# Iheckzza/FeatureMatching

Hardware: AMD Instinct MI355X
Metric: image-pairs/sec at 640x480 (coarse corr + dual-softmax mutual-NN + fine window refinement) (higher is better)
Workload: dtype i8 screening + f32 exact; 1 GPU; 640x480 pair, C=256 @1/8 (L=S=4800), Cf=64 @1/2, 5x5 fine window, 'peaky' descriptors; launch=hipGraph replay, concurrent_streams=4, fine_maps_layout=nchw

## Files before the change

featurematching_amd/csrc/fine.hip:

```cpp
#include "fm_device.h"
#include "fm_fine_device.h"
#include "fm_maps_device.h"

namespace fm {

__device__ __forceinline__ int xcd_contiguous(int bid, int n) {
  const int q = n >> 3, rem = n & 7, x = bid & 7, y = bid >> 3;
  return (x < rem ? x * (q + 1) : rem * (q + 1) + (x - rem) * q) + y;
}

typedef _Float16 half8 __attribute__((ext_vector_type(8)));
typedef float f32x16 __attribute__((ext_vector_type(16)));

constexpr float kMergeWgtScale = 4096.f;
__device__ __forceinline__ float merge_act_scale(float amax) {
  const unsigned bits = __float_as_uint(amax);
  const int e = (int)((bits >> 23) & 0xffu);
  int k = 140 - e;
  if (e == 255) k = 0;
  k = k > 40 ? 40 : (k < -100 ? -100 : k);
  return __uint_as_float((unsigned)(127 + k) << 23);
}
template <int W>
__device__ __forceinline__ void wave_merge_tile(float* tile, int lane, const half8* __restrict__ wpack,
                                                const float* __restrict__ ctx_row) {
  constexpr int WW = W * W, PITCH = 68, MT = (WW + 31) / 32;
  const int r = lane & 31, h = lane >> 5;
  const float c0 = ctx_row[r], c1 = ctx_row[32 + r];
  half8 bhi[2][4], blo[2][4];
#pragma unroll
  for (int nt = 0; nt < 2; ++nt)
#pragma unroll
    for (int ks = 0; ks < 4; ++ks) {
      bhi[nt][ks] = wpack[((nt * 4 + ks) * 2 + 0) * 64 + lane];
      blo[nt][ks] = wpack[((nt * 4 + ks) * 2 + 1) * 64 + lane];
    }
  float amax = 0.f;
#pragma unroll
  for (int mt = 0; mt < MT; ++mt) {
    const int row = min(32 * mt + r, WW - 1);
#pragma unroll
    for (int ks = 0; ks < 4; ++ks) {
      const float4 p = *reinterpret_cast<const float4*>(tile + row * PITCH + ks * 16 + 8 * h);
      const float4 q = *reinterpret_cast<const float4*>(tile + row * PITCH + ks * 16 + 8 * h + 4);
      amax = fmaxf(amax, fmaxf(fmaxf(fmaxf(fabsf(p.x), fabsf(p.y)), fmaxf(fabsf(p.z), fabsf(p.w))),
                               fmaxf(fmaxf(fabsf(q.x), fabsf(q.y)), fmaxf(fabsf(q.z), fabsf(q.w)))));
    }
  }
#pragma unroll
  for (int m = 32; m >= 1; m >>= 1) amax = fmaxf(amax, __shfl_xor(amax, m));
  const float act_scale = merge_act_scale(amax);
  half8 ahi[MT][4], alo[MT][4];
#pragma unroll
  for (int mt = 0; mt < MT; ++mt) {
    const int row = min(32 * mt + r, WW - 1);
#pragma unroll
    for (int ks = 0; ks < 4; ++ks) {
      const float4 p = *reinterpret_cast<const float4*>(tile + row * PITCH + ks * 16 + 8 * h);
      const float4 q = *reinterpret_cast<const float4*>(tile + row * PITCH + ks * 16 + 8 * h + 4);
      const float x[8] = {p.x, p.y, p.z, p.w, q.x, q.y, q.z, q.w};
#pragma unroll
      for (int e = 0; e < 8; ++e) {
        const float xs = x[e] * act_scale;
        const _Float16 hh = (_Float16)xs;
        ahi[mt][ks][e] = hh;
        alo[mt][ks][e] = (_Float16)(xs - (float)hh);
      }
    }
  }
  __builtin_amdgcn_wave_barrier();
  const float inv_scale = (1.0f / act_scale) * (1.0f / kMergeWgtScale);
#pragma unroll
  for (int mt = 0; mt < MT; ++mt) {
#pragma unroll
    for (int nt = 0; nt < 2; ++nt) {
      f32x16 acc;
#pragma unroll
      for (int g = 0; g < 16; ++g) acc[g] = (nt ? c1 : c0) * (act_scale * kMergeWgtScale);
#pragma unroll
      for (int ks = 0; ks < 4; ++ks) {
        acc = __builtin_amdgcn_mfma_f32_32x32x16_f16(ahi[mt][ks], bhi[nt][ks], acc, 0, 0, 0);
        acc = __builtin_amdgcn_mfma_f32_32x32x16_f16(alo[mt][ks], bhi[nt][ks], acc, 0, 0, 0);
        acc = __builtin_amdgcn_mfma_f32_32x32x16_f16(ahi[mt][ks], blo[nt][ks], acc, 0, 0, 0);
      }
#pragma unroll
      for (int g = 0; g < 16; ++g) {
        const int row = 32 * mt + (g & 3) + 8 * (g >> 2) + 4 * h;
        if (row < WW) tile[row * PITCH + 32 * nt + r] = acc[g] * inv_scale;
      }
    }
  }
  __builtin_amdgcn_wave_barrier();
}

template <int W>
__device__ __forceinline__ void wave_load_window64(const float* src, int Hf, int Wf, int oy, int ox, float* tile, int lane) {
  constexpr int CF = 64, WW = W * W, PITCH = CF + 4;
  constexpr int SLOTS = W == 5 ? 32 : 64, CPI = 64 / SLOTS, NLOAD = CF / CPI;
  static_assert(W == 5 || W == 7, "position decode below is for W in {5,7}");
  const int rem = lane & (SLOTS - 1), hi = lane / SLOTS;
  const int wy = W == 5 ? (rem * 13) >> 6 : (rem * 37) >> 8;
  const int wx = rem - wy * W;
  const int y = oy + wy, x = ox + wx;
  const bool ok = rem < WW && y >= 0 && y < Hf && x >= 0 && x < Wf;
  const __amdgpu_buffer_rsrc_t rsrc =
      __builtin_amdgcn_make_buffer_rsrc(const_cast<float*>(src), 0, CF * Hf * Wf * 4, 0x00020000);
  const unsigned voff = ok ? (unsigned)((hi * Hf + y) * Wf + x) * 4u : 0x80000000u;
  const int step = Hf * Wf * 4 * CPI;
  float v[NLOAD];
#pragma unroll
  for (int it = 0; it < NLOAD; ++it) {
#ifndef FM_ABL_G_NOLOAD
    v[it] = __builtin_bit_cast(float, __builtin_amdgcn_raw_buffer_load_b32(rsrc, voff, it * step, 0));
#else
    v[it] = 0.f;
#endif
  }
  float* slot = tile + rem * PITCH + hi;
#pragma unroll
  for (int it = 0; it < NLOAD; ++it)
    if (rem < WW) slot[it * CPI] = v[it];
  __builtin_amdgcn_wave_barrier();
}

template <int W>
__device__ __forceinline__ void wave_store_tile64(const float* tile, float* __restrict__ dst, int lane) {
  constexpr int CF = 64, WW = W * W, TOTAL = CF * WW, PITCH = CF + 4;
  float4* dst4 = reinterpret_cast<float4*>(dst);
#pragma unroll
  for (int it = 0; it < (TOTAL / 4 + 63) / 64; ++it) {
    const int idx = it * 64 + lane;
    if (idx < TOTAL / 4) {
      const float4 q = *reinterpret_cast<const float4*>(tile + (idx >> 4) * PITCH + (idx & 15) * 4);
#ifdef FM_ABL_G_NOSTORE
      if (q.x == 1.2345e-30f) dst4[idx] = q;
#else
      dst4[idx] = q;
#endif
    }
  }
  __builtin_amdgcn_wave_barrier();
}

template <int W, bool MERGE = false>
__device__ __forceinline__ void wave_copy_window64(const float* src, int Hf, int Wf, int oy, int ox,
                                                   float* __restrict__ dst, float* tile, int lane,
                                                   const half8* __restrict__ wpack = nullptr,
                                                   const float* __restrict__ ctx_row = nullptr) {
  wave_load_window64<W>(src, Hf, Wf, oy, ox, tile, lane);
  if (MERGE) wave_merge_tile<W>(tile, lane, wpack, ctx_row);
  wave_store_tile64<W>(tile, dst, lane);
}

constexpr int kGatherTileFloats(int W) { return W * W * 68; }

template <int W, bool MERGE>
__global__ __launch_bounds__(256) void k_gather_nchw64(const float* __restrict__ feat, int Hf, int Wf, int stride,
                                                       int pad, int w_c, const int64_t* __restrict__ b_ids,
                                                       const int64_t* __restrict__ ids,
                                                       const int32_t* __restrict__ d_count, int m_max,
                                                       float* __restrict__ out, const half8* __restrict__ wpack,
                                                       const float* __restrict__ ctx, int ctx_cells) {
  constexpr int CF = 64, TOTAL = CF * W * W;
  __shared__ __attribute__((aligned(16))) float tile[4 * kGatherTileFloats(W)];
  const int lane = threadIdx.x & 63, wv = __builtin_amdgcn_readfirstlane(threadIdx.x >> 6);
  const int M = d_count ? min(d_count[0], m_max) : m_max;
  const int per = (M + 7) >> 3;
  const int slot = (int)(blockIdx.x >> 3) * 4 + wv;
  const int m = (blockIdx.x & 7) * per + slot;
  if (slot >= per || m >= M) return;
  const int b = __builtin_amdgcn_readfirstlane((int)b_ids[m]);
  const int id = __builtin_amdgcn_readfirstlane((int)ids[m]);
  const int cy = id / w_c;
  wave_copy_window64<W, MERGE>(feat + (long)b * CF * Hf * Wf, Hf, Wf, cy * stride - pad, (id - cy * w_c) * stride - pad,
                               out + (long)m * TOTAL, tile + wv * kGatherTileFloats(W), lane, wpack,
                               MERGE ? ctx + ((long)b * ctx_cells + id) * CF : nullptr);
}

struct CellImage {
  const float* feat; int Hf, Wf, w_c, cells, total_cells;
  const int32_t* cell_to_match; int cell_pitch; const int32_t* ties;
  const int64_t* ids; float* out; const float* ctx;
};
struct CellArgs {
  CellImage im[2];
  int stride, pad, m_max;
  const int64_t* b_ids; const int32_t* d_count; const half8* wpack;
};

template <int W, bool MERGE>
__global__ __launch_bounds__(256) void k_gather_cellorder64(CellArgs a) {
  constexpr int CF = 64, TOTAL = CF * W * W;
  __shared__ __attribute__((aligned(16))) float tile_all[4 * kGatherTileFloats(W)];
  const CellImage& I = a.im[blockIdx.y];
  const int lane = threadIdx.x & 63, wv = __builtin_amdgcn_readfirstlane(threadIdx.x >> 6);
  float* tile = tile_all + wv * kGatherTileFloats(W);
  const int M = a.d_count ? min(a.d_count[0], a.m_max) : a.m_max;
  const int nties = I.ties[0];
  const int lid = xcd_contiguous(blockIdx.x, gridDim.x) * 4 + wv;
  int jm = -1, jb = 0, jcell = 0;
  if (lid < I.total_cells) {
    const int b = lid / I.cells, cell = lid - b * I.cells;
    const int m = I.cell_to_match[(long)b * I.cell_pitch + cell] - 1;
    if (m >= 0 && m < M) { jm = m; jb = b; jcell = cell; }
  }
  const int gwave = blockIdx.x * 4 + wv, nwaves = gridDim.x * 4;
  const int mode = nties == 0 ? 0 : (nties <= kTieCap ? 1 : 2);
  int q = gwave;
  const int chunk = (M + nwaves - 1) / nwaves;
  int scan = gwave * chunk;
  const int scan_end = min(M, scan + chunk);
  for (;;) {
    if (jm >= 0) {
      jm = __builtin_amdgcn_readfirstlane(jm); jb = __builtin_amdgcn_readfirstlane(jb);
      jcell = __builtin_amdgcn_readfirstlane(jcell);
      const int cy = jcell / I.w_c;
      wave_copy_window64<W, MERGE>(I.feat + (long)jb * CF * I.Hf * I.Wf, I.Hf, I.Wf, cy * a.stride - a.pad,
                                   (jcell - cy * I.w_c) * a.stride - a.pad, I.out + (long)jm * TOTAL, tile, lane,
                                   a.wpack, MERGE ? I.ctx + ((long)jb * I.cells + jcell) * CF : nullptr);
    }
    jm = -1;
    if (mode == 0) break;
    if (mode == 1) {
      if (q >= nties) break;
      const int m = I.ties[1 + q];
      q += nwaves;
      if (m >= 0 && m < M) { jm = m; jb = (int)a.b_ids[m]; jcell = (int)I.ids[m]; }
    } else {
      if (scan >= scan_end) break;
      const int m = scan++;
      const int mb = (int)a.b_ids[m], id = (int)I.ids[m];
      if (I.cell_to_match[(long)mb * I.cell_pitch + id] != m + 1) { jm = m; jb = mb; jcell = id; }
    }
  }
}

template <int DT> struct MapElem { using type = float; };
template <> struct MapElem<FM_F16> { using type = unsigned short; };
template <> struct MapElem<FM_BF16> { using type = unsigned short; };
template <int DT>
__device__ __forceinline__ float map_value(const typename MapElem<DT>::type* p, long i) {
  if constexpr (DT == FM_F32) return p[i];
  else return half_bits_to_float(p[i], DT);
}

template <int DT>
__global__ __launch_bounds__(256) void k_gather_nchw(const typename MapElem<DT>::type* __restrict__ feat, int Cf, int Hf, int Wf, int W,
                                                     int stride, int pad, int w_c, const int64_t* __restrict__ b_ids,
                                                     const int64_t* __restrict__ ids, const int32_t* __restrict__ d_count,
                                                     int m_max, float* __restrict__ out) {
  extern __shared__ __attribute__((aligned(16))) float tile[];
  const int m = blockIdx.x;
  const int M = d_count ? min(d_count[0], m_max) : m_max;
  if (m >= M) return;
  const int WW = W * W;
  const int b = (int)b_ids[m];
  const int id = (int)ids[m];
  const int oy = (id / w_c) * stride - pad;
  const int ox = (id % w_c) * stride - pad;
  const typename MapElem<DT>::type* src = feat + (long)b * Cf * Hf * Wf;
  const int total = Cf * WW;
  for (int idx = threadIdx.x; idx < total; idx += 256) {
    const int c = idx / WW;
    const int rem = idx - c * WW;
    const int wy = rem / W, wx = rem - wy * W;
    const int y = oy + wy, x = ox + wx;
    float v = 0.f;
    if (y >= 0 && y < Hf && x >= 0 && x < Wf) v = map_value<DT>(src, ((long)c * Hf + y) * Wf + x);
    tile[rem * (Cf + 1) + c] = v;
  }
  __syncthreads();
  float* dst = out + (long)m * total;
  for (int idx = threadIdx.x; idx < total; idx += 256) {
    const int rpos = idx / Cf;
    const int c = idx - rpos * Cf;
    dst[idx] = tile[rpos * (Cf + 1) + c];
  }
}

template <int DT>
__global__ __launch_bounds__(256) void k_gather_nhwc(const typename MapElem<DT>::type* __restrict__ feat, int Cf, int Hf, int Wf, int W,
                                                     int stride, int pad, int w_c, const int64_t* __restrict__ b_ids,
                                                     const int64_t* __restrict__ ids, const int32_t* __restrict__ d_count,
                                                     int m_max, float* __restrict__ out) {
  const int m = blockIdx.x;
  const int M = d_count ? min(d_count[0], m_max) : m_max;
  if (m >= M) return;
  const int WW = W * W;
  const int b = (int)b_ids[m];
  const int id = (int)ids[m];
  const int oy = (id / w_c) * stride - pad;
  const int ox = (id % w_c) * stride - pad;
  const int c4 = Cf / 4;
  const typename MapElem<DT>::type* src = feat + (long)b * Hf * Wf * Cf;
  float4* dst = reinterpret_cast<float4*>(out + (long)m * WW * Cf);
  for (int idx = threadIdx.x; idx < WW * c4; idx += 256) {
    const int rpos = idx / c4;
    const int c = idx - rpos * c4;
    const int wy = rpos / W, wx = rpos - wy * W;
    const int y = oy + wy, x = ox + wx;
    float4 v = make_float4(0.f, 0.f, 0.f, 0.f);
    if (y >= 0 && y < Hf && x >= 0 && x < Wf) {
      const long e = ((long)y * Wf + x) * c4 + c;
      if constexpr (DT == FM_F32) v = reinterpret_cast<const float4*>(src)[e];
      else v = half4_to_float4(reinterpret_cast<const uint2*>(src)[e], DT);
    }
    dst[idx] = v;
  }
}


template <int W>
__device__ __forceinline__ void soft_argmax2(float sim0, float sim1, int pos, bool on, int lane, float inv_sqrt_c,
                                             float scale_f, float k0x, float k0y, float k1x, float k1y, float* out0,
                                             float* out1) {
  const Heat2 e = heat_exp2(sim0, sim1, on, inv_sqrt_c);
  const float t = heat_sums2<W>(e.e0, e.e1, pos);
  auto sum_k = [&](int k) { return heat_sum(t, k); };
  if (lane == 0) {
    float* const outs[2] = {out0, out1};
    const float kx[2] = {k0x, k1x}, ky[2] = {k0y, k1y};
#pragma unroll
    for (int d = 0; d < 2; ++d) {
      const float inv = 1.0f / sum_k(5 * d);
      const float cx = sum_k(5 * d + 1) * inv, cy = sum_k(5 * d + 2) * inv;
      const float vx = sum_k(5 * d + 3) * inv - cx * cx, vy = sum_k(5 * d + 4) * inv - cy * cy;
      outs[d][0] = kx[d] + (cx * (float)(W / 2) * scale_f + (float)(W / 2));
      outs[d][1] = ky[d] + (cy * (float)(W / 2) * scale_f + (float)(W / 2));
      outs[d][2] = sqrtf(fmaxf(vx, 1e-10f)) + sqrtf(fmaxf(vy, 1e-10f));
    }
  }
}

template <int W>
__device__ __forceinline__ void fine_core(const float (&f0)[W * W], const float (&f1)[W * W], int lane,
                                          const float* __restrict__ mix0, const float* __restrict__ mix1, float k0x,
                                          float k0y, float k1x, float k1y, float scale_f, float* __restrict__ out0,
                                          float* __restrict__ out1) {
  constexpr int WW = W * W;
  constexpr int CF = 64;
  const Mix2 q = fine_mix<W>(f0, f1, mix0, mix1);
  const float q0 = q.q0, q1 = q.q1;

#ifdef FM_ABL_F_NOCOMPUTE
  if (q0 + q1 == 1.2345e-30f) out0[0] = q0;
  return;
#endif
  const float inv_sqrt_c = 1.0f / sqrtf((float)CF);
  constexpr int NP = WW > 32 ? 64 : 32;
  float p[NP];
#pragma unroll
  for (int r = 0; r < NP; ++r) p[r] = r < WW ? q0 * f1[r] : 0.f;
  const float sim0 = transpose_reduce<NP>(p, lane);
#pragma unroll
  for (int r = 0; r < NP; ++r) p[r] = r < WW ? q1 * f0[r] : 0.f;
  const float sim1 = transpose_reduce<NP>(p, lane);

  const int pos = tr_index<NP>(lane);
  const bool on = pos < WW && (NP == 64 || !(lane & 1));
  soft_argmax2<W>(sim0, sim1, pos, on, lane, inv_sqrt_c, scale_f, k0x, k0y, k1x, k1y, out0, out1);
}

template <int W>
__global__ __launch_bounds__(256) void k_fine(const float* __restrict__ win0, const float* __restrict__ win1, int m_max,
                                              const int32_t* __restrict__ d_count, const float* __restrict__ mix0,
                                              const float* __restrict__ mix1, const float* __restrict__ kc0,
                                              const float* __restrict__ kc1, float scale_f, float* __restrict__ out0,
                                              float* __restrict__ out1) {
  constexpr int WW = W * W;
  constexpr int CF = 64;
  const int lane = threadIdx.x & 63;
  const int m = blockIdx.x * 4 + (threadIdx.x >> 6);
  const int M = d_count ? min(d_count[0], m_max) : m_max;
  if (m >= M) return;
  const float* p0 = win0 + (long)m * WW * CF + lane;
  const float* p1 = win1 + (long)m * WW * CF + lane;
  float f0[WW], f1[WW];
#pragma unroll
  for (int r = 0; r < WW; ++r) { f0[r] = __builtin_nontemporal_load(p0 + r * CF); f1[r] = __builtin_nontemporal_load(p1 + r * CF); }
  fine_core<W>(f0, f1, lane, mix0, mix1, kc0[m * 2], kc0[m * 2 + 1], kc1[m * 2], kc1[m * 2 + 1], scale_f,
               out0 + (long)m * 3, out1 + (long)m * 3);
}

template <int W>
__global__ __launch_bounds__(256) void k_gather_nhwc64(const float* __restrict__ feat, int Hf, int Wf, int stride, int pad,
                                                       int w_c, const int64_t* __restrict__ b_ids,
                                                       const int64_t* __restrict__ ids, const int32_t* __restrict__ d_count,
                                                       int m_max, float* __restrict__ out) {
  constexpr int ROW16 = W * 16;
  constexpr int TOTAL16 = W * ROW16;
  constexpr int NIT = (TOTAL16 + 63) / 64;
  const int lane = threadIdx.x & 63, wv = __builtin_amdgcn_readfirstlane(threadIdx.x >> 6);
  const int M = d_count ? min(d_count[0], m_max) : m_max;
  const int per = (M + 7) >> 3;
  const int slot = (int)(blockIdx.x >> 3) * 4 + wv;
  const int m = (blockIdx.x & 7) * per + slot;
  if (slot >= per || m >= M) return;
  const int b = __builtin_amdgcn_readfirstlane((int)b_ids[m]);
  const int id = __builtin_amdgcn_readfirstlane((int)ids[m]);
  const int cy = id / w_c;
  const int oy = cy * stride - pad, ox = (id - cy * w_c) * stride - pad;
  const float4* src = reinterpret_cast<const float4*>(feat + (long)b * Hf * Wf * 64);
  float4* dst = reinterpret_cast<float4*>(out + (long)m * W * W * 64);
  float4 v[NIT];
#pragma unroll
  for (int it = 0; it < NIT; ++it) {
    const int k = it * 64 + lane;
    const int wy = k / ROW16, within = k - wy * ROW16;
    const int y = oy + wy, x = ox + (within >> 4);
    const bool ok = k < TOTAL16 && y >= 0 && y < Hf && x >= 0 && x < Wf;
    const float4 t = src[ok ? ((long)y * Wf + x) * 16 + (within & 15) : 0];
    v[it] = ok ? t : make_float4(0.f, 0.f, 0.f, 0.f);
  }
#pragma unroll
  for (int it = 0; it < NIT; ++it) {
    const int k = it * 64 + lane;
    if (k < TOTAL16) dst[k] = v[it];
  }
}

struct MergeNhwcImage {
  const void* feat; int Hf, Wf, w_c, cells;
  const int64_t* ids; float* out; const float* ctx;
};
struct MergeNhwcArgs {
  MergeNhwcImage im[2];
  int stride, pad, m_max;
  const int64_t* b_ids; const int32_t* d_count; const half8* wpack;
};

template <int W, int DT>
__global__ __launch_bounds__(256) void k_gather_merge_nhwc64(MergeNhwcArgs a) {
  constexpr int WW = W * W, PITCH = 68;
  constexpr int TOTAL16 = WW * 16;
  constexpr int NIT = (TOTAL16 + 63) / 64;
  using Chunk = typename std::conditional<DT == FM_F32, float4, uint2>::type;
  __shared__ __attribute__((aligned(16))) float tile_all[4 * kGatherTileFloats(W)];
  const MergeNhwcImage& I = a.im[blockIdx.y];
  const int lane = threadIdx.x & 63, wv = __builtin_amdgcn_readfirstlane(threadIdx.x >> 6);
  float* tile = tile_all + wv * kGatherTileFloats(W);
  const int M = a.d_count ? min(a.d_count[0], a.m_max) : a.m_max;
  const int per = (M + 7) >> 3;
  const int slot = (int)(blockIdx.x >> 3) * 4 + wv;
  const int m = (blockIdx.x & 7) * per + slot;
  if (slot >= per || m >= M) return;
  const int b = __builtin_amdgcn_readfirstlane((int)a.b_ids[m]);
  const int id = __builtin_amdgcn_readfirstlane((int)I.ids[m]);
  const int cy = id / I.w_c;
  const int oy = cy * a.stride - a.pad, ox = (id - cy * I.w_c) * a.stride - a.pad;
  const Chunk* src = reinterpret_cast<const Chunk*>(I.feat) + (long)b * I.Hf * I.Wf * 16;
  Chunk v[NIT];
#pragma unroll
  for (int it = 0; it < NIT; ++it) {
    const int k = it * 64 + lane;
    const int pos = k >> 4, wy = pos / W;
    const int y = oy + wy, x = ox + (pos - wy * W);
    const bool ok = k < TOTAL16 && y >= 0 && y < I.Hf && x >= 0 && x < I.Wf;
    const Chunk t = src[ok ? ((long)y * I.Wf + x) * 16 + (k & 15) : 0];
    if constexpr (DT == FM_F32) v[it] = ok ? t : make_float4(0.f, 0.f, 0.f, 0.f);
    else v[it] = ok ? t : make_uint2(0u, 0u);
  }
#pragma unroll
  for (int it = 0; it < NIT; ++it) {
    const int k = it * 64 + lane;
    if (k < TOTAL16) {
      float4* slot4 = reinterpret_cast<float4*>(tile + (k >> 4) * PITCH + (k & 15) * 4);
      if constexpr (DT == FM_F32) *slot4 = v[it];
      else *slot4 = half4_to_float4(v[it], DT);
    }
  }
  __builtin_amdgcn_wave_barrier();
  wave_merge_tile<W>(tile, lane, a.wpack, I.ctx + ((long)b * I.cells + id) * 64);
  wave_store_tile64<W>(tile, I.out + (long)m * WW * 64, lane);
}

template <int W, bool NCHW0, int DT = FM_F32>
__global__ __launch_bounds__(256) void k_fine_maps(const float* __restrict__ map0, const float* __restrict__ map1, int Hf0,
                                                   int Wf0, int Hf1, int Wf1, int stride, int pad, int w0c, int w1c,
                                                   const int64_t* __restrict__ b_ids, const int64_t* __restrict__ i_ids,
                                                   const int64_t* __restrict__ j_ids, const int32_t* __restrict__ d_count,
                                                   int m_max, const float* __restrict__ mix0, const float* __restrict__ mix1,
                                                   const float* __restrict__ kc0, const float* __restrict__ kc1, float scale_f,
                                                   float* __restrict__ out0, float* __restrict__ out1) {
  constexpr int WW = W * W;
  const int lane = threadIdx.x & 63, wv = __builtin_amdgcn_readfirstlane(threadIdx.x >> 6);
  const int M = d_count ? min(d_count[0], m_max) : m_max;
  const int per = (M + 7) >> 3;
  __shared__ __attribute__((aligned(16))) float tile_all[NCHW0 ? 4 * kGatherTileFloats(W) : 4];
  for (int slot = (int)(blockIdx.x >> 3) * 4 + wv; slot < per; slot += (int)(gridDim.x >> 3) * 4) {
  const int m = (blockIdx.x & 7) * per + slot;
  if (m >= M) break;
  const int b = __builtin_amdgcn_readfirstlane((int)b_ids[m]);
  const int i = __builtin_amdgcn_readfirstlane((int)i_ids[m]);
  const int j = __builtin_amdgcn_readfirstlane((int)j_ids[m]);
  const int cy0 = i / w0c, cy1 = j / w1c;
  const int oy0 = cy0 * stride - pad, ox0 = (i - cy0 * w0c) * stride - pad;
  const int oy1 = cy1 * stride - pad, ox1 = (j - cy1 * w1c) * stride - pad;
  constexpr int EB = DT == FM_F32 ? 4 : 2;
  constexpr int PXB = 64 * EB;
  static_assert(!(NCHW0 && DT != FM_F32), "half-precision maps are read channels-last");
  const char* base0 = reinterpret_cast<const char*>(map0) + (long)b * Hf0 * Wf0 * PXB;
  const char* base1 = reinterpret_cast<const char*>(map1) + (long)b * Hf1 * Wf1 * PXB;
  unsigned vo0[W], vo1[W];
#pragma unroll
  for (int wx = 0; wx < W; ++wx) {
    const int x0 = ox0 + wx, x1 = ox1 + wx;
    vo0[wx] = x0 >= 0 ? (unsigned)(x0 * PXB + lane * EB) : 0x80000000u;
    vo1[wx] = x1 >= 0 ? (unsigned)(x1 * PXB + lane * EB) : 0x80000000u;
  }
  auto load_elem = [](const __amdgpu_buffer_rsrc_t r, unsigned vo) -> float {
    if constexpr (DT == FM_F32) return __builtin_bit_cast(float, __builtin_amdgcn_raw_buffer_load_b32(r, vo, 0, 0));
    else return half_bits_to_float((unsigned)(unsigned short)__builtin_amdgcn_raw_buffer_load_b16(r, vo, 0, 0), DT);
  };
  float f0[WW], f1[WW];
#pragma unroll
  for (int wy = 0; wy < W; ++wy) {
    const int y0 = oy0 + wy, y1 = oy1 + wy;
    const bool ok0 = y0 >= 0 && y0 < Hf0, ok1 = y1 >= 0 && y1 < Hf1;
    const __amdgpu_buffer_rsrc_t r1 = __builtin_amdgcn_make_buffer_rsrc(
        const_cast<char*>(base1 + (long)(ok1 ? y1 : 0) * Wf1 * PXB), 0, ok1 ? Wf1 * PXB : 0, 0x00020000);
    if (!NCHW0) {
      const __amdgpu_buffer_rsrc_t r0 = __builtin_amdgcn_make_buffer_rsrc(
          const_cast<char*>(base0 + (long)(ok0 ? y0 : 0) * Wf0 * PXB), 0, ok0 ? Wf0 * PXB : 0, 0x00020000);
#pragma unroll
      for (int wx = 0; wx < W; ++wx) f0[wy * W + wx] = load_elem(r0, vo0[wx]);
    }
#pragma unroll
    for (int wx = 0; wx < W; ++wx) f1[wy * W + wx] = load_elem(r1, vo1[wx]);
  }
  if (NCHW0) {
    float* tile = tile_all + wv * kGatherTileFloats(W);
    wave_load_window64<W>(reinterpret_cast<const float*>(base0), Hf0, Wf0, oy0, ox0, tile, lane);
#pragma unroll
    for (int r = 0; r < WW; ++r) f0[r] = tile[r * 68 + lane];
  }
  fine_core<W>(f0, f1, lane, mix0, mix1, kc0[m * 2], kc0[m * 2 + 1], kc1[m * 2], kc1[m * 2 + 1], scale_f,
               out0 + (long)m * 3, out1 + (long)m * 3);
  }
}


template <typename T>
__global__ __launch_bounds__(256) void k_nchw_to_nhwc64(const T* __restrict__ src, T* __restrict__ dst, int Hf, int Wf,
                                                        int N) {
  __shared__ T tile[64 * 65];
  nchw_to_nhwc64_units<T>(src, dst, Hf, Wf, N, tile, blockIdx.x, gridDim.x);
}

}

using namespace fm;

template <bool MERGE>
static void launch_list64(int W, int blocks, hipStream_t st, const float* feat_f, int Hf, int Wf, int stride, int pad,
                          int w_c, const int64_t* b_ids, const int64_t* ids, const int32_t* d_count, int m_max,
                          float* out, const half8* wpack, const float* ctx, int ctx_cells) {
  with_window(W, [&](auto w) {
    hipLaunchKernelGGL((k_gather_nchw64<decltype(w)::value, MERGE>), dim3(blocks), dim3(256), 0, st, feat_f, Hf, Wf, stride,
                       pad, w_c, b_ids, ids, d_count, m_max, out, wpack, ctx, ctx_cells);
  });
}
static CellImage cell_image(const float* feat, int N, int Hf, int Wf, int h_c, int w_c, const int32_t* map, int pitch,
                            const int32_t* ties, const int64_t* ids, float* out, const float* ctx) {
  CellImage im;
  im.feat = feat; im.Hf = Hf; im.Wf = Wf; im.w_c = w_c; im.cells = h_c * w_c; im.total_cells = N * h_c * w_c;
  im.cell_to_match = map; im.cell_pitch = pitch; im.ties = ties; im.ids = ids; im.out = out; im.ctx = ctx;
  return im;
}
static CellArgs cell_args(const CellImage& im0, const CellImage& im1, int stride, int pad, int m_max, const int64_t* b_ids,
                          const int32_t* d_count, const void* packed_w) {
  CellArgs a;
  a.im[0] = im0; a.im[1] = im1;
  a.stride = stride; a.pad = pad; a.m_max = m_max; a.b_ids = b_ids; a.d_count = d_count; a.wpack = (const half8*)packed_w;
  return a;
}
static bool fast_nchw64(int Cf, int Hf, int Wf, int W) {
  return Cf == 64 && (W == 5 || W == 7) && (long)Hf * Wf * 64 * 4 < (1L << 31);
}
static int list_blocks(int m_max) { return 8 * (((m_max + 7) / 8 + 3) / 4); }
constexpr int kFineGridCap = 1 << 20;
static int cell_blocks(long total) { return (int)(((total + 3) / 4 + 7) / 8 * 8); }
static int launch_cells64(int W, int nimg, long total, const CellArgs& a, hipStream_t st) {
  with_window(W, [&](auto w) {
    auto launch = [&](auto merge) {
      hipLaunchKernelGGL((k_gather_cellorder64<decltype(w)::value, decltype(merge)::value>), dim3(cell_blocks(total), nimg),
                         dim3(256), 0, st, a);
    };
    if (a.wpack) launch(std::true_type{});
    else launch(std::false_type{});
  });
  return (int)hipGetLastError();
}

template <int DT>
static void launch_generic_gather(const void* feat_f, int Cf, int Hf, int Wf, int layout, int W, int stride, int pad, int w_c,
                                  const int64_t* b_ids, const int64_t* ids, const int32_t* d_count, int m_max, float* out,
                                  hipStream_t st) {
  using E = typename MapElem<DT>::type;
  if (layout == 0) {
    const size_t smem = (size_t)W * W * (Cf + 1) * sizeof(float);
    hipLaunchKernelGGL(k_gather_nchw<DT>, dim3(m_max), dim3(256), smem, st, (const E*)feat_f, Cf, Hf, Wf, W, stride, pad, w_c,
                       b_ids, ids, d_count, m_max, out);
  } else {
    hipLaunchKernelGGL(k_gather_nhwc<DT>, dim3(m_max), dim3(256), 0, st, (const E*)feat_f, Cf, Hf, Wf, W, stride, pad, w_c,
                       b_ids, ids, d_count, m_max, out);
  }
}

extern "C" int fm_gather_windows_dtype(const void* feat_f, int map_dtype, int N, int Cf, int Hf, int Wf, int layout, int W,
                                       int stride, int pad, int w_c, const int64_t* b_ids, const int64_t* ids,
                                       const int32_t* d_count, int m_max, float* out, void* stream) {
  if (m_max == 0) return FM_OK;
  if (!feat_f || !b_ids || !ids || !out) return FM_E_NULL;
  if (map_dtype != FM_F32 && map_dtype != FM_F16 && map_dtype != FM_BF16) return FM_E_UNSUPPORTED;
  if (!crop_shape_ok(N, Hf, Wf, stride, m_max) || Cf <= 0 || W <= 0 || w_c <= 0) return FM_E_SHAPE;
  if (W > 15 || Cf > 512 || (layout == 1 && Cf % 4) || (layout != 0 && layout != 1)) return FM_E_UNSUPPORTED;
  hipStream_t st = (hipStream_t)stream;
  if (layout == 0 && (size_t)W * W * (Cf + 1) * sizeof(float) > 64 * 1024 &&
      !(map_dtype == FM_F32 && fast_nchw64(Cf, Hf, Wf, W))) return FM_E_UNSUPPORTED;
  if (map_dtype == FM_F32 && layout == 0 && fast_nchw64(Cf, Hf, Wf, W)) {
    launch_list64<false>(W, list_blocks(m_max), st, (const float*)feat_f, Hf, Wf, stride, pad, w_c, b_ids, ids, d_count, m_max,
                         out, nullptr, nullptr, 0);
  } else if (map_dtype == FM_F32 && layout == 1 && Cf == 64 && (W == 5 || W == 7)) {
    with_window(W, [&](auto w) {
      hipLaunchKernelGGL(k_gather_nhwc64<decltype(w)::value>, dim3(list_blocks(m_max)), dim3(256), 0, st,
                         (const float*)feat_f, Hf, Wf, stride, pad, w_c, b_ids, ids, d_count, m_max, out);
    });
  } else if (map_dtype == FM_F32) {
    launch_generic_gather<FM_F32>(feat_f, Cf, Hf, Wf, layout, W, stride, pad, w_c, b_ids, ids, d_count, m_max, out, st);
  } else if (map_dtype == FM_F16) {
    launch_generic_gather<FM_F16>(feat_f, Cf, Hf, Wf, layout, W, stride, pad, w_c, b_ids, ids, d_count, m_max, out, st);
  } else {
    launch_generic_gather<FM_BF16>(feat_f, Cf, Hf, Wf, layout, W, stride, pad, w_c, b_ids, ids, d_count, m_max, out, st);
  }
  return (int)hipGetLastError();
}

extern "C" int fm_gather_windows(const float* feat_f, int N, int Cf, int Hf, int Wf, int layout, int W, int stride,
                                 int pad, int w_c, const int64_t* b_ids, const int64_t* ids, const int32_t* d_count,
                                 int m_max, float* out, void* stream) {
  return fm_gather_windows_dtype(feat_f, FM_F32, N, Cf, Hf, Wf, layout, W, stride, pad, w_c, b_ids, ids, d_count, m_max, out,
                                 stream);
}

extern "C" int fm_gather_windows_cells(const float* feat_f, int N, int Cf, int Hf, int Wf, int W, int stride, int pad,
                                       int h_c, int w_c, const int32_t* cell_to_match, int cell_pitch,
                                       const int32_t* ties, const int64_t* b_ids, const int64_t* ids,
                                       const int32_t* d_count, int m_max, float* out, void* stream) {
  if (m_max == 0) return FM_OK;
  if (!feat_f || !cell_to_match || !ties || !b_ids || !ids || !out) return FM_E_NULL;
  if (!crop_shape_ok(N, Hf, Wf, stride, m_max) || h_c <= 0 || w_c <= 0 || cell_pitch < h_c * w_c) return FM_E_SHAPE;
  if (!fast_nchw64(Cf, Hf, Wf, W)) return FM_E_UNSUPPORTED;
  const CellImage im = cell_image(feat_f, N, Hf, Wf, h_c, w_c, cell_to_match, cell_pitch, ties, ids, out, nullptr);
  return launch_cells64(W, 1, (long)N * h_c * w_c, cell_args(im, im, stride, pad, m_max, b_ids, d_count, nullptr),
                        (hipStream_t)stream);
}

__global__ __launch_bounds__(256) void k_merge_pack(const float* __restrict__ merge_w, half8* __restrict__ packed) {
  const int idx = blockIdx.x * 256 + threadIdx.x;
  if (idx >= 512) return;
  const int lane = idx & 63, ks = (idx >> 6) & 3, nt = idx >> 8;
  const float* src = merge_w + (32 * nt + (lane & 31)) * 128 + 16 * ks + 8 * (lane >> 5);
  half8 hh, ll;
#pragma unroll
  for (int j = 0; j < 8; ++j) {
    float x = src[j] * kMergeWgtScale;
    if (!(fabsf(x) <= 65504.f)) x = __builtin_nanf("");
    hh[j] = (_Float16)x;
    ll[j] = (_Float16)(x - (float)hh[j]);
  }
  packed[((nt * 4 + ks) * 2 + 0) * 64 + lane] = hh;
  packed[((nt * 4 + ks) * 2 + 1) * 64 + lane] = ll;
}

extern "C" int fm_merge_pack_weights(const float* merge_w, int Cf, void* packed, void* stream) {
  if (!merge_w || !packed) return FM_E_NULL;
  if (Cf != 64) return FM_E_UNSUPPORTED;
  hipLaunchKernelGGL(k_merge_pack, dim3(2), dim3(256), 0, (hipStream_t)stream, merge_w, (half8*)packed);
  return (int)hipGetLastError();
}

extern "C" int fm_gather_merge_windows(const float* feat_f, int N, int Cf, int Hf, int Wf, int W, int stride, int pad,
                                       int h_c, int w_c, const int32_t* cell_to_match, int cell_pitch,
                                       const int32_t* ties, const void* packed_w, const float* ctx_bias,
                                       const int64_t* b_ids, const int64_t* ids, const int32_t* d_count, int m_max,
                                       float* out, void* stream) {
  if (m_max == 0) return FM_OK;
  if (!feat_f || !packed_w || !ctx_bias || !b_ids || !ids || !out) return FM_E_NULL;
  if (cell_to_match && !ties) return FM_E_NULL;
  if (!crop_shape_ok(N, Hf, Wf, stride, m_max) || h_c <= 0 || w_c <= 0 || (cell_to_match && cell_pitch < h_c * w_c))
    return FM_E_SHAPE;
  if (!fast_nchw64(Cf, Hf, Wf, W)) return FM_E_UNSUPPORTED;
  hipStream_t st = (hipStream_t)stream;
  if (cell_to_match) {
    const CellImage im = cell_image(feat_f, N, Hf, Wf, h_c, w_c, cell_to_match, cell_pitch, ties, ids, out, ctx_bias);
    return launch_cells64(W, 1, (long)N * h_c * w_c, cell_args(im, im, stride, pad, m_max, b_ids, d_count, packed_w), st);
  }
  launch_list64<true>(W, list_blocks(m_max), st, feat_f, Hf, Wf, stride, pad, w_c, b_ids, ids, d_count, m_max, out,
                      (const half8*)packed_w, ctx_bias, h_c * w_c);
  return (int)hipGetLastError();
}

extern "C" int fm_gather_windows_pair(const float* feat_f0, const float* feat_f1, int N, int Cf, int Hf0, int Wf0,
                                      int Hf1, int Wf1, int W, int stride, int pad, int h0c, int w0c, int h1c, int w1c,
                                      const int32_t* cell0, int pitch0, const int32_t* ties0, const int32_t* cell1,
                                      int pitch1, const int32_t* ties1, const void* packed_w, const float* ctx0,
                                      const float* ctx1, const int64_t* b_ids, const int64_t* i_ids,
                                      const int64_t* j_ids, const int32_t* d_count, int m_max, float* out0,
                                      float* out1, void* stream) {
  if (m_max == 0) return FM_OK;
  if (!feat_f0 || !feat_f1 || !cell0 || !cell1 || !ties0 || !ties1 || !b_ids || !i_ids || !j_ids || !out0 || !out1)
    return FM_E_NULL;
  if (packed_w && (!ctx0 || !ctx1)) return FM_E_NULL;
  if (!crop_shape_ok(N, Hf0, Wf0, stride, m_max) || !crop_shape_ok(N, Hf1, Wf1, stride, m_max) || h0c <= 0 || w0c <= 0 ||
      h1c <= 0 || w1c <= 0 || pitch0 < h0c * w0c || pitch1 < h1c * w1c)
    return FM_E_SHAPE;
  if (!fast_nchw64(Cf, Hf0, Wf0, W) || !fast_nchw64(Cf, Hf1, Wf1, W)) return FM_E_UNSUPPORTED;
  const CellArgs a = cell_args(cell_image(feat_f0, N, Hf0, Wf0, h0c, w0c, cell0, pitch0, ties0, i_ids, out0, ctx0),
                               cell_image(feat_f1, N, Hf1, Wf1, h1c, w1c, cell1, pitch1, ties1, j_ids, out1, ctx1), stride,
                               pad, m_max, b_ids, d_count, packed_w);
  const long t0 = (long)N * h0c * w0c, t1 = (long)N * h1c * w1c;
  return launch_cells64(W, 2, t0 > t1 ? t0 : t1, a, (hipStream_t)stream);
}

static MergeNhwcImage merge_nhwc_image(const void* feat, int Hf, int Wf, int h_c, int w_c, const int64_t* ids, float* out,
                                       const float* ctx) {
  MergeNhwcImage im;
  im.feat = feat; im.Hf = Hf; im.Wf = Wf; im.w_c = w_c; im.cells = h_c * w_c; im.ids = ids; im.out = out; im.ctx = ctx;
  return im;
}

extern "C" int fm_gather_merge_windows_nhwc(const void* feat_f0, const void* feat_f1, int map_dtype, int N, int Cf, int Hf0,
                                            int Wf0, int Hf1, int Wf1, int W, int stride, int pad, int h0c, int w0c,
                                            int h1c, int w1c, const void* packed_w, const float* ctx0, const float* ctx1,
                                            const int64_t* b_ids, const int64_t* i_ids, const int64_t* j_ids,
                                            const int32_t* d_count, int m_max, float* out0, float* out1, void* stream) {
  if (m_max == 0) return FM_OK;
  const bool pair = feat_f1 != nullptr;
  if (!feat_f0 || !packed_w || !ctx0 || !b_ids || !i_ids || !out0) return FM_E_NULL;
  if (pair && (!ctx1 || !j_ids || !out1)) return FM_E_NULL;
  if (!crop_shape_ok(N, Hf0, Wf0, stride, m_max) || h0c <= 0 || w0c <= 0) return FM_E_SHAPE;
  if (pair && (!crop_shape_ok(N, Hf1, Wf1, stride, m_max) || h1c <= 0 || w1c <= 0)) return FM_E_SHAPE;
  if (map_dtype != FM_F32 && map_dtype != FM_F16 && map_dtype != FM_BF16) return FM_E_UNSUPPORTED;
  if (Cf != 64 || (W != 5 && W != 7)) return FM_E_UNSUPPORTED;
  MergeNhwcArgs a;
  a.im[0] = merge_nhwc_image(feat_f0, Hf0, Wf0, h0c, w0c, i_ids, out0, ctx0);
  a.im[1] = pair ? merge_nhwc_image(feat_f1, Hf1, Wf1, h1c, w1c, j_ids, out1, ctx1) : a.im[0];
  a.stride = stride; a.pad = pad; a.m_max = m_max; a.b_ids = b_ids; a.d_count = d_count; a.wpack = (const half8*)packed_w;
  with_window(W, [&](auto w) {
    auto launch = [&](auto dt) {
      hipLaunchKernelGGL((k_gather_merge_nhwc64<decltype(w)::value, decltype(dt)::value>),
                         dim3(list_blocks(m_max), pair ? 2 : 1), dim3(256), 0, (hipStream_t)stream, a);
    };
    if (map_dtype == FM_F16) launch(int_c<FM_F16>{});
    else if (map_dtype == FM_BF16) launch(int_c<FM_BF16>{});
    else launch(int_c<FM_F32>{});
  });
  return (int)hipGetLastError();
}

extern "C" int fm_fine_match(const float* win0, const float* win1, int m_max, const int32_t* d_count, int WW, int Cf,
                             const float* mix0, const float* mix1, const float* mkpts0_c, const float* mkpts1_c,
                             float scale_f, float* out0, float* out1, void* stream) {
  if (m_max == 0) return FM_OK;
  if (!win0 || !win1 || !mix0 || !mix1 || !mkpts0_c || !mkpts1_c || !out0 || !out1) return FM_E_NULL;
  if (m_max < 0) return FM_E_SHAPE;
  if (Cf != 64 || (WW != 25 && WW != 49)) return FM_E_UNSUPPORTED;
  hipStream_t st = (hipStream_t)stream;
  const int blocks = (m_max + 3) / 4;
  with_window(WW == 25 ? 5 : 7, [&](auto w) {
    hipLaunchKernelGGL(k_fine<decltype(w)::value>, dim3(blocks), dim3(256), 0, st, win0, win1, m_max, d_count, mix0, mix1,
                       mkpts0_c, mkpts1_c, scale_f, out0, out1);
  });
  return (int)hipGetLastError();
}

struct FineMapsScratch { Span map[2]; size_t total; };
static FineMapsScratch fine_maps_layout(int N, int Cf, int Hf0, int Wf0, int Hf1, int Wf1, int map_dtype) {
  const size_t elem = map_dtype == FM_F32 ? 4 : 2;
  FineMapsScratch s;
  s.map[0] = {0, map_dtype == FM_F32 ? 0 : (size_t)N * Cf * elem * (size_t)Hf0 * Wf0};
  s.map[1] = {align256(s.map[0].bytes), (size_t)N * Cf * elem * (size_t)Hf1 * Wf1};
  s.total = s.map[1].at + s.map[1].bytes;
  return s;
}

extern "C" size_t fm_fine_maps_scratch_bytes_dtype(int N, int Cf, int Hf0, int Wf0, int Hf1, int Wf1, int layout, int map_dtype) {
  if (layout != 0 || N <= 0 || Cf <= 0 || Hf0 <= 0 || Wf0 <= 0 || Hf1 <= 0 || Wf1 <= 0) return 0;
  return fine_maps_layout(N, Cf, Hf0, Wf0, Hf1, Wf1, map_dtype).total;
}

template <typename T>
static void launch_channels_last_copy(const void* src, void* dst, int N, int Hf, int Wf, int grid_cap, hipStream_t st) {
  const long pieces = (long)((Wf + 63) / 64) * Hf * N;
  hipLaunchKernelGGL(k_nchw_to_nhwc64<T>, dim3((unsigned)(pieces < grid_cap ? pieces : grid_cap)), dim3(256), 0, st,
                     (const T*)src, (T*)dst, Hf, Wf, N);
}
extern "C" size_t fm_fine_maps_scratch_bytes(int N, int Cf, int Hf0, int Wf0, int Hf1, int Wf1, int layout) {
  return fm_fine_maps_scratch_bytes_dtype(N, Cf, Hf0, Wf0, Hf1, Wf1, layout, FM_F32);
}

extern "C" int fm_fine_match_maps_dtype(const void* feat_f0, const void* feat_f1, int map_dtype, int layout, int N, int Cf,
                                        int Hf0, int Wf0, int Hf1, int Wf1, int W, int stride, int pad, int w0c, int w1c,
                                        const int64_t* b_ids, const int64_t* i_ids, const int64_t* j_ids,
                                        const int32_t* d_count, int m_max, const float* mix0, const float* mix1,
                                        const float* mkpts0_c, const float* mkpts1_c, float scale_f, void* scratch,
                                        float* out0, float* out1, void* stream) {
  if (m_max == 0) return FM_OK;
  if (!feat_f0 || !feat_f1 || !b_ids || !i_ids || !j_ids || !mix0 || !mix1 || !mkpts0_c || !mkpts1_c || !out0 || !out1)
    return FM_E_NULL;
  if (!crop_shape_ok(N, Hf0, Wf0, stride, m_max) || !crop_shape_ok(N, Hf1, Wf1, stride, m_max) || w0c <= 0 || w1c <= 0)
    return FM_E_SHAPE;
  if (map_dtype != FM_F32 && map_dtype != FM_F16 && map_dtype != FM_BF16) return FM_E_UNSUPPORTED;
  if ((layout != 0 && layout != 1 && layout != FM_LAYOUT_NCHW_PREPARED) || !fast_nchw64(Cf, Hf0, Wf0, W) ||
      !fast_nchw64(Cf, Hf1, Wf1, W))
    return FM_E_UNSUPPORTED;
  const bool prepared = layout == FM_LAYOUT_NCHW_PREPARED;
  if (prepared && map_dtype != FM_F32) return FM_E_UNSUPPORTED;
  if (prepared) layout = 0;
  if (layout == 0 && !scratch) return FM_E_NULL;
  hipStream_t st = (hipStream_t)stream;
  const float* m0 = (const float*)feat_f0;
  const float* m1 = (const float*)feat_f1;
  int grid_cap = kFineGridCap;
#ifdef FM_TUNE_ENV
  if (const char* e = getenv("FM_FINE_GRID")) grid_cap = atoi(e) > 0 ? atoi(e) / 8 * 8 : kFineGridCap;
#endif
  if (layout == 0) {
    const FineMapsScratch sc = fine_maps_layout(N, Cf, Hf0, Wf0, Hf1, Wf1, map_dtype);
    float* s0 = span_ptr<float>(scratch, sc.map[0]);
    float* s1 = span_ptr<float>(scratch, sc.map[1]);
    if (map_dtype == FM_F32) {
      if (!prepared) launch_channels_last_copy<float>(feat_f1, s1, N, Hf1, Wf1, grid_cap, st);
    } else {
      launch_channels_last_copy<unsigned short>(feat_f0, s0, N, Hf0, Wf0, grid_cap, st);
      launch_channels_last_copy<unsigned short>(feat_f1, s1, N, Hf1, Wf1, grid_cap, st);
      m0 = s0;
    }
    m1 = s1;
  }
  const int blocks = list_blocks(m_max) < grid_cap ? list_blocks(m_max) : grid_cap;
  with_window(W, [&](auto w) {
    auto launch = [&](auto nchw0, auto dt) {
      hipLaunchKernelGGL((k_fine_maps<decltype(w)::value, decltype(nchw0)::value, decltype(dt)::value>), dim3(blocks),
                         dim3(256), 0, st, m0, m1, Hf0, Wf0, Hf1, Wf1, stride, pad, w0c, w1c, b_ids, i_ids, j_ids, d_count,
                         m_max, mix0, mix1, mkpts0_c, mkpts1_c, scale_f, out0, out1);
    };
    if (map_dtype == FM_F16) launch(std::false_type{}, int_c<FM_F16>{});
    else if (map_dtype == FM_BF16) launch(std::false_type{}, int_c<FM_BF16>{});
    else if (layout == 0) launch(std::true_type{}, int_c<FM_F32>{});
    else launch(std::false_type{}, int_c<FM_F32>{});
  });
  return (int)hipGetLastError();
}

extern "C" int fm_fine_match_maps(const float* feat_f0, const float* feat_f1, int layout, int N, int Cf, int Hf0, int Wf0,
                                  int Hf1, int Wf1, int W, int stride, int pad, int w0c, int w1c, const int64_t* b_ids,
                                  const int64_t* i_ids, const int64_t* j_ids, const int32_t* d_count, int m_max,
                                  const float* mix0, const float* mix1, const float* mkpts0_c, const float* mkpts1_c,
                                  float scale_f, void* scratch, float* out0, float* out1, void* stream) {
  return fm_fine_match_maps_dtype(feat_f0, feat_f1, FM_F32, layout, N, Cf, Hf0, Wf0, Hf1, Wf1, W, stride, pad, w0c, w1c,
                                  b_ids, i_ids, j_ids, d_count, m_max, mix0, mix1, mkpts0_c, mkpts1_c, scale_f, scratch,
                                  out0, out1, stream);
}
```

Before: 20370 image-pairs/s.

## Batch adjacent fine matches into shared strip loads for NCHW 5x5 windows

For the NCHW f32 path with a 5x5 window, consecutive matches whose coarse indices are horizontally adjacent in image 0 are processed together as a run. One overlapping strip of the image-0 map is loaded into LDS with 64-bit buffer loads and reused across the run's windows. Runs that fail the adjacency, stride, parity or alignment checks fall back to per-match processing, and the launch grid is sized by the number of runs. The change adds per-wave control flow, a larger LDS tile and more registers for the extra image-1 windows. Any gain depends on how often adjacent matches actually occur.

```diff
diff --git a/featurematching_amd/csrc/fine.hip b/featurematching_amd/csrc/fine.hip
--- a/featurematching_amd/csrc/fine.hip
+++ b/featurematching_amd/csrc/fine.hip
@@ -120,6 +120,44 @@
 #pragma unroll
   for (int it = 0; it < NLOAD; ++it)
     if (rem < WW) slot[it * CPI] = v[it];
+  __builtin_amdgcn_wave_barrier();
+}
+
+constexpr int kRunStride = 4;
+constexpr int kStripPitch = 65;
+constexpr int kStripPixels(int W, int R) { return kRunStride * (R - 1) + W; }
+constexpr int kStripTileFloats(int W, int R) { return W * kStripPixels(W, R) * kStripPitch; }
+
+template <int W, int R>
+__device__ __forceinline__ void wave_load_strip64(const float* src, int Hf, int Wf, int oy, int ox, float* tile, int lane) {
+  constexpr int CF = 64, SP = kStripPixels(W, R), NX2 = (SP + 1) / 2, USED = W * NX2;
+  constexpr int SLOTS = USED <= 32 ? 32 : 64, CPI = 64 / SLOTS, NLOAD = CF / CPI;
+  static_assert(USED <= 64, "one strip of one channel per wave-load at most");
+  const int rem = lane & (SLOTS - 1), hi = lane / SLOTS;
+  const int wy = rem / NX2, k = rem - wy * NX2;
+  const int y = oy + wy, x = ox + 2 * k;
+  const bool ok = rem < USED && y >= 0 && y < Hf && x >= 0 && x + 1 < Wf;
+  const __amdgpu_buffer_rsrc_t rsrc =
+      __builtin_amdgcn_make_buffer_rsrc(const_cast<float*>(src), 0, CF * Hf * Wf * 4, 0x00020000);
+  const unsigned voff = ok ? (unsigned)((hi * Hf + y) * Wf + x) * 4u : 0x80000000u;
+  const int step = Hf * Wf * 4 * CPI;
+  unsigned long long v[NLOAD];
+#pragma unroll
+  for (int it = 0; it < NLOAD; ++it) {
+#ifndef FM_ABL_G_NOLOAD
+    v[it] = __builtin_bit_cast(unsigned long long, __builtin_amdgcn_raw_buffer_load_b64(rsrc, voff, it * step, 0));
+#else
+    v[it] = 0ull;
+#endif
+  }
+  float* slot = tile + (wy * SP + 2 * k) * kStripPitch + hi;
+  const bool second = 2 * k + 1 < SP;
+#pragma unroll
+  for (int it = 0; it < NLOAD; ++it)
+    if (rem < USED) {
+      slot[it * CPI] = __uint_as_float((unsigned)v[it]);
+      if (second) slot[kStripPitch + it * CPI] = __uint_as_float((unsigned)(v[it] >> 32));
+    }
   __builtin_amdgcn_wave_barrier();
 }
 
@@ -474,6 +512,107 @@
   wave_store_tile64<W>(tile, I.out + (long)m * WW * 64, lane);
 }
 
+
+#ifndef FM_FINE_RUN
+#define FM_FINE_RUN 2
+#endif
+constexpr int kFineRun(int W, bool nchw0) { return nchw0 && W == 5 ? FM_FINE_RUN : 1; }
+constexpr int kFineMapsTileFloats(int W, bool nchw0) {
+  return !nchw0 ? 1
+                : (kFineRun(W, nchw0) > 1 && kStripTileFloats(W, kFineRun(W, nchw0)) > kGatherTileFloats(W)
+                       ? kStripTileFloats(W, kFineRun(W, nchw0))
+                       : kGatherTileFloats(W));
+}
+
+struct FineMapsArgs {
+  const float *__restrict__ map0, *__restrict__ map1;
+  int Hf0, Wf0, Hf1, Wf1, stride, pad, w0c, w1c;
+  const int64_t *__restrict__ b_ids, *__restrict__ i_ids, *__restrict__ j_ids;
+  const float *__restrict__ mix0, *__restrict__ mix1, *__restrict__ kc0, *__restrict__ kc1;
+  float scale_f;
+  float *__restrict__ out0, *__restrict__ out1;
+};
+
+template <int W, int R>
+__device__ __forceinline__ void fine_maps_unit(const FineMapsArgs& a, int m, int b, int i, const int (&js)[R], float* tile,
+                                               int lane) {
+  constexpr int WW = W * W;
+  const int stride = a.stride, pad = a.pad, Hf1 = a.Hf1, Wf1 = a.Wf1;
+  const int cy0 = i / a.w0c;
+  const int oy0 = cy0 * stride - pad, ox0 = (i - cy0 * a.w0c) * stride - pad;
+  const float* base0 = a.map0 + (long)b * a.Hf0 * a.Wf0 * 64;
+  const char* base1 = reinterpret_cast<const char*>(a.map1) + (long)b * Hf1 * Wf1 * 256;
+  float f1[R][WW];
+#pragma unroll
+  for (int t = 0; t < R; ++t) {
+    const int cy1 = js[t] / a.w1c;
+    const int oy1 = cy1 * stride - pad, ox1 = (js[t] - cy1 * a.w1c) * stride - pad;
+    unsigned vo1[W];
+#pragma unroll
+    for (int wx = 0; wx < W; ++wx) vo1[wx] = ox1 + wx >= 0 ? (unsigned)((ox1 + wx) * 256 + lane * 4) : 0x80000000u;
+#pragma unroll
+    for (int wy = 0; wy < W; ++wy) {
+      const int y1 = oy1 + wy;
+      const bool ok1 = y1 >= 0 && y1 < Hf1;
+      const __amdgpu_buffer_rsrc_t r1 = __builtin_amdgcn_make_buffer_rsrc(
+          const_cast<char*>(base1 + (long)(ok1 ? y1 : 0) * Wf1 * 256), 0, ok1 ? Wf1 * 256 : 0, 0x00020000);
+#pragma unroll
+      for (int wx = 0; wx < W; ++wx)
+        f1[t][wy * W + wx] = __builtin_bit_cast(float, __builtin_amdgcn_raw_buffer_load_b32(r1, vo1[wx], 0, 0));
+    }
+  }
+  constexpr int PITCH = R > 1 ? kStripPitch : 68, SP = R > 1 ? kStripPixels(W, R) : W;
+  if constexpr (R > 1) wave_load_strip64<W, R>(base0, a.Hf0, a.Wf0, oy0, ox0, tile, lane);
+  else wave_load_window64<W>(base0, a.Hf0, a.Wf0, oy0, ox0, tile, lane);
+#pragma unroll
+  for (int t = 0; t < R; ++t) {
+    float f0[WW];
+#pragma unroll
+    for (int r = 0; r < WW; ++r) f0[r] = tile[((r / W) * SP + (r % W) + t * kRunStride) * PITCH + lane];
+    const int mt = m + t;
+    fine_core<W>(f0, f1[t], lane, a.mix0, a.mix1, a.kc0[mt * 2], a.kc0[mt * 2 + 1], a.kc1[mt * 2], a.kc1[mt * 2 + 1],
+                 a.scale_f, a.out0 + (long)mt * 3, a.out1 + (long)mt * 3);
+  }
+  __builtin_amdgcn_wave_barrier();
+}
+
+template <int W, int RUN>
+__device__ __forceinline__ void fine_maps_runs(const FineMapsArgs& a, int M, float* tile, int lane, int wv) {
+  const int per = (M + 7) >> 3;
+  const int m_lo = (blockIdx.x & 7) * per, m_hi = min(m_lo + per, M);
+  for (int slot = (int)(blockIdx.x >> 3) * 4 + wv; m_lo + slot * RUN < m_hi; slot += (int)(gridDim.x >> 3) * 4) {
+    const int m = m_lo + slot * RUN;
+    const int n = min(RUN, m_hi - m);
+    const int b = __builtin_amdgcn_readfirstlane((int)a.b_ids[m]);
+    const int i = __builtin_amdgcn_readfirstlane((int)a.i_ids[m]);
+    const int cx0 = i % a.w0c;
+    bool run = n == RUN && cx0 + RUN <= a.w0c && a.stride == kRunStride && !((cx0 * a.stride - a.pad) & 1) &&
+               !(a.Wf0 & 1) && !((unsigned)(size_t)a.map0 & 7u);
+    int js[RUN];
+#pragma unroll
+    for (int t = 0; t < RUN; ++t) js[t] = 0;
+    if (run) {
+      js[0] = __builtin_amdgcn_readfirstlane((int)a.j_ids[m]);
+#pragma unroll
+      for (int t = 1; t < RUN; ++t) {
+        run = run && __builtin_amdgcn_readfirstlane((int)a.b_ids[m + t]) == b &&
+              __builtin_amdgcn_readfirstlane((int)a.i_ids[m + t]) == i + t;
+        js[t] = __builtin_amdgcn_readfirstlane((int)a.j_ids[m + t]);
+      }
+    }
+    if (run) {
+      fine_maps_unit<W, RUN>(a, m, b, i, js, tile, lane);
+    } else {
+#pragma unroll 1
+      for (int t = 0; t < n; ++t) {
+        const int j1[1] = {__builtin_amdgcn_readfirstlane((int)a.j_ids[m + t])};
+        fine_maps_unit<W, 1>(a, m + t, __builtin_amdgcn_readfirstlane((int)a.b_ids[m + t]),
+                             __builtin_amdgcn_readfirstlane((int)a.i_ids[m + t]), j1, tile, lane);
+      }
+    }
+  }
+}
+
 template <int W, bool NCHW0, int DT = FM_F32>
 __global__ __launch_bounds__(256) void k_fine_maps(const float* __restrict__ map0, const float* __restrict__ map1, int Hf0,
                                                    int Wf0, int Hf1, int Wf1, int stride, int pad, int w0c, int w1c,
@@ -486,7 +625,13 @@
   const int lane = threadIdx.x & 63, wv = __builtin_amdgcn_readfirstlane(threadIdx.x >> 6);
   const int M = d_count ? min(d_count[0], m_max) : m_max;
   const int per = (M + 7) >> 3;
-  __shared__ __attribute__((aligned(16))) float tile_all[NCHW0 ? 4 * kGatherTileFloats(W) : 4];
+  __shared__ __attribute__((aligned(16))) float tile_all[NCHW0 ? 4 * kFineMapsTileFloats(W, NCHW0) : 4];
+  if constexpr (kFineRun(W, NCHW0) > 1) {
+    const FineMapsArgs a = {map0, map1, Hf0, Wf0, Hf1, Wf1, stride, pad, w0c, w1c, b_ids, i_ids, j_ids,
+                            mix0, mix1, kc0, kc1, scale_f, out0, out1};
+    fine_maps_runs<W, kFineRun(W, NCHW0)>(a, M, tile_all + wv * kFineMapsTileFloats(W, NCHW0), lane, wv);
+    return;
+  }
   for (int slot = (int)(blockIdx.x >> 3) * 4 + wv; slot < per; slot += (int)(gridDim.x >> 3) * 4) {
   const int m = (blockIdx.x & 7) * per + slot;
   if (m >= M) break;
@@ -839,7 +984,9 @@
     }
     m1 = s1;
   }
-  const int blocks = list_blocks(m_max) < grid_cap ? list_blocks(m_max) : grid_cap;
+  const int run = kFineRun(W, map_dtype == FM_F32 && layout == 0);
+  const int units = list_blocks((m_max + run - 1) / run);
+  const int blocks = units < grid_cap ? units : grid_cap;
   with_window(W, [&](auto w) {
     auto launch = [&](auto nchw0, auto dt) {
       hipLaunchKernelGGL((k_fine_maps<decltype(w)::value, decltype(nchw0)::value, decltype(dt)::value>), dim3(blocks),
```

After: 19800 image-pairs/s. 0.972x the previous value.
